# UmaimaKhan01/SkyEye-Aerial-Object-Detection-using-Yolo

Measured on AMD Instinct MI355X. Metric: frames/sec @1280x1280 + p50 latency, skyeye_s 1-GPU and skyeye_l 8-GPU, higher is better.
Workload: dtype bf16

## Files before the change

### skyeye-aerial-object-detection-using-yolo_amd/csrc/k_csp_stage.hip

```cpp
#include "sky_kernels.h"

#include "conv_frag.h"

namespace sky {

namespace cs {
constexpr int NW = 8, NT = NW * 64;
constexpr int TS = 16, HW = TS + 2, NHP = HW * HW;
constexpr int C = 64, HD = 32;
constexpr int XPIX = 352, XPL = XPIX * 32, X_BYTES = 4 * XPL;
constexpr int XDMA = XPIX / 32;
constexpr int HSL = 336, HPLN = HSL * 16, H_BYTES = 4 * HPLN;
constexpr int CPLN = 256 * 16, C_BYTES = 4 * CPLN;
constexpr int NFR = (NHP + 15) / 16;
constexpr int W12_BYTES = 2 * C * 64, WB1_BYTES = 1 * HD * 64, WB2_BYTES = 9 * HD * 64, W3_BYTES = 2 * C * 64;
constexpr int LDS_BYTES = X_BYTES + 2 * H_BYTES + C_BYTES + W12_BYTES + WB1_BYTES + WB2_BYTES + W3_BYTES + (C + HD + HD + C) * 4;
static_assert(LDS_BYTES <= 160 * 1024, "one workgroup per CU");
static_assert(HPLN % 256 == 0 && CPLN % 256 == 0 && XPL % 256 == 0, "planes a multiple of 256 B apart: conflict-free fragment reads");
}

__device__ __forceinline__ void cs_wait_vmcnt0() { __builtin_amdgcn_s_waitcnt(0x0F70); }
__device__ __forceinline__ void cs_lds_dma16(__amdgpu_buffer_rsrc_t rsrc, char* dst, int voff)
{
    __builtin_amdgcn_raw_ptr_buffer_load_lds(rsrc, (__attribute__((address_space(3))) void*)dst, 16, voff, 0, 0, 0);
}

template <int ROWS, int KSTEPS>
__device__ __forceinline__ void cs_stage_weights(const void* w, int kpad, char* lds, int tid)
{
    const char* src = reinterpret_cast<const char*>(w);
    for (int idx = tid; idx < KSTEPS * ROWS * 4; idx += cs::NT) {
        const int ks = idx / (ROWS * 4), rc = idx - ks * (ROWS * 4);
        const int rowp = rc >> 2, c = rc & 3;
        const int j = rowp >> 4, r = rowp & 15;
        const int ch = (j >> 1) * 32 + (r >> 2) * 8 + (j & 1) * 4 + (r & 3);
        const u32x4_t v = *reinterpret_cast<const u32x4_t*>(src + (long)ch * kpad * 2 + ks * 64 + c * 16);
        *reinterpret_cast<u32x4_t*>(lds + ks * (ROWS * 64) + rowp * 64 + ((c ^ (((r >> 3) & 1) << 1)) << 4)) = v;
    }
}

__global__ void __launch_bounds__(cs::NT) csp_stage_kernel(const CspStageArgs a)
{
    using namespace cs;
    extern __shared__ __attribute__((aligned(1024))) char smem[];
    char* const xt = smem;
    char* const y1t = xt + X_BYTES;
    char* const ut = y1t + H_BYTES;
    char* const y2t = ut + H_BYTES;
    char* const w12 = y2t + C_BYTES;
    char* const wb1 = w12 + W12_BYTES;
    char* const wb2 = wb1 + WB1_BYTES;
    char* const w3 = wb2 + WB2_BYTES;
    float* const b12 = reinterpret_cast<float*>(w3 + W3_BYTES);
    float* const bb1 = b12 + C;
    float* const bb2 = bb1 + HD;
    float* const b3 = bb2 + HD;

#ifdef SKY_AB_WAVE_VECTOR
    const int tid = threadIdx.x, lane = tid & 63, wave = tid >> 6;
#else
    const int tid = threadIdx.x, lane = tid & 63, wave = __builtin_amdgcn_readfirstlane(tid >> 6);
#endif
    const int fr = lane & 15, fq = lane >> 4;
    const int tiles_x = (a.W + TS - 1) / TS, tiles_y = (a.H + TS - 1) / TS;
    const int ntile = a.B * tiles_y * tiles_x;
    int tile, tstep, tend;
    tile_walk(ntile, tile, tstep, tend);
    if (tile >= tend) return;
    const int pix_b = a.ldi * 2;

    cs_stage_weights<C, 2>(a.w12, a.kpad12, w12, tid);
    cs_stage_weights<HD, 1>(a.wb1, a.kpadb1, wb1, tid);
    cs_stage_weights<HD, 9>(a.wb2, a.kpadb2, wb2, tid);
    cs_stage_weights<C, 2>(a.w3, a.kpad3, w3, tid);
    for (int i = tid; i < C; i += NT) { b12[i] = a.b12[i]; b3[i] = a.b3[i]; }
    for (int i = tid; i < HD; i += NT) { bb1[i] = a.bb1[i]; bb2[i] = a.bb2[i]; }

    const __amdgpu_buffer_rsrc_t irsrc = __builtin_amdgcn_make_buffer_rsrc(const_cast<void*>(a.in), 0, (int)a.in_bytes, 0x00020000);
    auto decode_tile = [&](int t, int& bimg, int& y0, int& x0) {
        const int tx = t % tiles_x;
        const int q = t / tiles_x;
        bimg = q / tiles_y;
        y0 = (q - bimg * tiles_y) * TS;
        x0 = tx * TS;
    };
    auto issue_x = [&](int bimg, int y0, int x0) {
        const int pl = wave & 3;
        const int base = ((bimg * a.H + y0 - 1) * a.W + x0 - 1) * pix_b + pl * 16;
        const int b0 = wave < 4 ? 0 : 6, b1 = wave < 4 ? 6 : XDMA;
        for (int b = b0; b < b1; ++b) {
            const int p = b * 32 + (lane >> 1);
            const int hy = (p * 3641) >> 16, hx = p - hy * HW;
            const int kk = (lane & 1) ^ ((p >> 3) & 1);
            const bool ok = p < NHP && (unsigned)(y0 - 1 + hy) < (unsigned)a.H && (unsigned)(x0 - 1 + hx) < (unsigned)a.W;
            cs_lds_dma16(irsrc, xt + pl * XPL + b * 1024, ok ? base + (hy * a.W + hx) * pix_b + kk * 64 : -1);
        }
    };
    const int aswz = ((fq ^ (((fr >> 3) & 1) << 1)) << 4);
    auto wfrag = [&](const char* w, int rows, int ks, int j) -> u32x4_t {
        return *reinterpret_cast<const u32x4_t*>(w + ks * (rows * 64) + (j * 16 + fr) * 64 + aswz);
    };
    auto xfrag = [&](int p, int kk) -> u32x4_t {
        return *reinterpret_cast<const u32x4_t*>(xt + fq * XPL + p * 32 + ((kk ^ ((p >> 3) & 1)) << 4));
    };
    auto act_pack = [&](const f32x4_t& a0, const f32x4_t& a1, float (&v)[8]) {
#pragma unroll
        for (int e = 0; e < 4; ++e) {
            v[e] = S1<__bf16>::silu(a0[e]);
            v[4 + e] = S1<__bf16>::silu(a1[e]);
        }
    };
    auto bias_pair = [&](const float* bias, f32x4_t& a0, f32x4_t& a1) {
        a0 = *reinterpret_cast<const f32x4_t*>(bias + fq * 8);
        a1 = *reinterpret_cast<const f32x4_t*>(bias + fq * 8 + 4);
    };

    int bimg, y0, x0;
    decode_tile(tile, bimg, y0, x0);
    __syncthreads();
#ifdef SKY_AB_SETPRIO
    if (__builtin_amdgcn_readfirstlane(tid >> 6) >= 4) __builtin_amdgcn_s_setprio(1);
#endif
    issue_x(bimg, y0, x0);
    for (;;) {
        cs_wait_vmcnt0();
        __syncthreads();
#pragma unroll 1
        for (int f = wave; f < NFR; f += NW) {
            const int p = f * 16 + fr;
            const int pc = p < NHP ? p : NHP - 1;
            const u32x4_t x0f = xfrag(pc, 0), x1f = xfrag(pc, 1);
            f32x4_t acc0, acc1;
            bias_pair(b12, acc0, acc1);
            S1<__bf16>::mma(wfrag(w12, C, 0, 0), x0f, acc0);
            S1<__bf16>::mma(wfrag(w12, C, 0, 1), x0f, acc1);
            S1<__bf16>::mma(wfrag(w12, C, 1, 0), x1f, acc0);
            S1<__bf16>::mma(wfrag(w12, C, 1, 1), x1f, acc1);
            float v[8];
            act_pack(acc0, acc1, v);
            const Out8<__bf16>::raw_t y1v = Out8<__bf16>::pack(v, 1.0f);
            f32x4_t au0, au1;
            bias_pair(bb1, au0, au1);
            S1<__bf16>::mma(wfrag(wb1, HD, 0, 0), y1v.a, au0);
            S1<__bf16>::mma(wfrag(wb1, HD, 0, 1), y1v.a, au1);
            act_pack(au0, au1, v);
            Out8<__bf16>::raw_t uv = Out8<__bf16>::pack(v, 1.0f);
            const int hy = (pc * 3641) >> 16, hx = pc - hy * HW;
            const bool inside = (unsigned)(y0 - 1 + hy) < (unsigned)a.H && (unsigned)(x0 - 1 + hx) < (unsigned)a.W;
            if (!inside) uv.a = u32x4_t{0u, 0u, 0u, 0u};
            if (p < NHP) {
                *reinterpret_cast<u32x4_t*>(y1t + fq * HPLN + p * 16) = y1v.a;
                *reinterpret_cast<u32x4_t*>(ut + fq * HPLN + p * 16) = uv.a;
            }
        }
#pragma unroll
        for (int i = 0; i < 2; ++i) {
            const int r = 2 * wave + i;
            const int p = (r + 1) * HW + 1 + fr;
            const u32x4_t x0f = xfrag(p, 0), x1f = xfrag(p, 1);
            f32x4_t acc0, acc1;
            bias_pair(b12 + HD, acc0, acc1);
            S1<__bf16>::mma(wfrag(w12, C, 0, 2), x0f, acc0);
            S1<__bf16>::mma(wfrag(w12, C, 0, 3), x0f, acc1);
            S1<__bf16>::mma(wfrag(w12, C, 1, 2), x1f, acc0);
            S1<__bf16>::mma(wfrag(w12, C, 1, 3), x1f, acc1);
            float v[8];
            act_pack(acc0, acc1, v);
            *reinterpret_cast<u32x4_t*>(y2t + fq * CPLN + (r * 16 + fr) * 16) = Out8<__bf16>::pack(v, 1.0f).a;
        }
        __syncthreads();
        const int next = tile + tstep;
        int nb = 0, ny0 = 0, nx0 = 0;
        if (next < tend) {
            decode_tile(next, nb, ny0, nx0);
            issue_x(nb, ny0, nx0);
        }
        {
            f32x4_t acc[2][2];
#pragma unroll
            for (int i = 0; i < 2; ++i) bias_pair(bb2, acc[0][i], acc[1][i]);
#pragma unroll
            for (int tap = 0; tap < 9; ++tap) {
                const int ky = tap / 3, kx = tap - ky * 3;
                u32x4_t pf[2];
#pragma unroll
                for (int i = 0; i < 2; ++i) pf[i] = *reinterpret_cast<const u32x4_t*>(ut + fq * HPLN + ((2 * wave + i + ky) * HW + fr + kx) * 16);
#pragma unroll
                for (int j = 0; j < 2; ++j) {
                    const u32x4_t wf = wfrag(wb2, HD, tap, j);
#pragma unroll
                    for (int i = 0; i < 2; ++i) S1<__bf16>::mma(wf, pf[i], acc[j][i]);
                }
            }
            f32x4_t acc3[4][2];
#pragma unroll
            for (int s = 0; s < 2; ++s)
#pragma unroll
                for (int i = 0; i < 2; ++i) bias_pair(b3 + s * 32, acc3[2 * s][i], acc3[2 * s + 1][i]);
            u32x4_t vv[2], y2v[2];
#pragma unroll
            for (int i = 0; i < 2; ++i) {
                const int r = 2 * wave + i;
                float v[8];
                if (a.shortcut) {
                    const Out8<__bf16>::raw_t rv = Out8<__bf16>::load(y1t + fq * HPLN + ((r + 1) * HW + 1 + fr) * 16);
#pragma unroll
                    for (int e = 0; e < 8; ++e) {
                        const float xx = e < 4 ? acc[0][i][e] : acc[1][i][e - 4];
                        const float t = S1<__bf16>::gate(xx);
                        const float res = (e & 1) ? __uint_as_float(rv.a[e >> 1] & 0xffff0000u) : __uint_as_float(rv.a[e >> 1] << 16);
                        v[e] = __builtin_fmaf(xx, t, res);
                    }
                } else {
                    act_pack(acc[0][i], acc[1][i], v);
                }
                vv[i] = Out8<__bf16>::pack(v, 1.0f).a;
                y2v[i] = *reinterpret_cast<const u32x4_t*>(y2t + fq * CPLN + (r * 16 + fr) * 16);
            }
#pragma unroll
            for (int j = 0; j < 4; ++j) {
                const u32x4_t wf = wfrag(w3, C, 0, j);
#pragma unroll
                for (int i = 0; i < 2; ++i) S1<__bf16>::mma(wf, vv[i], acc3[j][i]);
            }
#pragma unroll
            for (int j = 0; j < 4; ++j) {
                const u32x4_t wf = wfrag(w3, C, 1, j);
#pragma unroll
                for (int i = 0; i < 2; ++i) S1<__bf16>::mma(wf, y2v[i], acc3[j][i]);
            }
#pragma unroll
            for (int i = 0; i < 2; ++i) {
                const int oy = y0 + 2 * wave + i, ox = x0 + fr;
                if (oy < a.H && ox < a.W) {
                    char* op = reinterpret_cast<char*>(a.out) + (((long)bimg * a.H + oy) * a.W + ox) * (long)a.ldo * 2;
#pragma unroll
                    for (int s = 0; s < 2; ++s) {
                        float v[8];
                        act_pack(acc3[2 * s][i], acc3[2 * s + 1][i], v);
                        Out8<__bf16>::store(Out8<__bf16>::pack(v, 1.0f), op + (s * 32 + fq * 8) * 2);
                    }
                }
            }
        }
        if (next >= tend) break;
        tile = next; bimg = nb; y0 = ny0; x0 = nx0;
    }
}

bool csp_stage_supported(const CspStageArgs& a)
{
    return a.c == cs::C && a.hidden == cs::HD && a.ldi % 8 == 0 && a.ldo % 8 == 0 && a.in_bytes != 0 && a.kpad12 >= cs::C && a.kpadb1 >= cs::HD &&
           a.kpadb2 >= 9 * cs::HD && a.kpad3 >= cs::C && a.H >= 1 && a.W >= 1 && !(a.opts & OPT_NO_CSP_STAGE);
}

hipError_t launch_csp_stage(const CspStageArgs& a, hipStream_t s)
{
    if (!csp_stage_supported(a)) return hipErrorNotSupported;
    static size_t attr[16] = {0};
    {
        const hipError_t e = ensure_lds_attr(reinterpret_cast<const void*>(csp_stage_kernel), cs::LDS_BYTES, a.device, attr);
        if (e != hipSuccess) return e;
    }
    const int ntile = a.B * ((a.H + cs::TS - 1) / cs::TS) * ((a.W + cs::TS - 1) / cs::TS);
    const int n_cu = a.n_cu > 0 ? a.n_cu : 256;
    const int gx = ntile < n_cu ? ntile : n_cu;
    hipLaunchKernelGGL(csp_stage_kernel, dim3(gx), dim3(cs::NT), cs::LDS_BYTES, s, a);
    return hipGetLastError();
}

}
```

### skyeye-aerial-object-detection-using-yolo_amd/csrc/k_stem_down.hip

```cpp
#include "sky_kernels.h"

#include "conv_frag.h"

namespace sky {

namespace sd {
constexpr int NW = 8;
constexpr int NT = NW * 64;
constexpr int C1 = 32, C2 = 64;
constexpr int TS = 16;
constexpr int SS = 2 * TS + 1;
constexpr int HS = SS + 2;
constexpr int RS = 2 * HS;
constexpr int RDW = (2 * HS + 2) / 4;
constexpr int RAWP = RDW * 4;
constexpr int RAW_BYTES = 3 * RS * RAWP;
constexpr int NDW = (3 * RS * RDW + NT - 1) / NT;
constexpr int S2D_SLOTS = (HS * HS + 15) / 16 * 16;
constexpr int S2D_PLANE = S2D_SLOTS * 16;
constexpr int S2D_BYTES = 2 * S2D_PLANE;
constexpr int NPIX = (S2D_SLOTS + NT - 1) / NT;
constexpr int PC00 = 304, PC01 = 272, PC10 = 272, PC11 = 256;
constexpr int PB00 = 0, PB01 = PB00 + 4 * PC00 * 16 + 64, PB10 = PB01 + 4 * PC01 * 16 + 64, PB11 = PB10 + 4 * PC10 * 16 + 64;
constexpr int STEM_BYTES = PB11 + 4 * PC11 * 16 + 64;
static_assert(PB00 % 128 == 0 && PB10 % 128 == 0 && PB01 % 128 == 64 && PB11 % 128 == 64, "odd-column planes 64 bytes off the even ones");
static_assert(STEM_BYTES % 256 == 0, "the space-to-depth tile behind the stem tile stays 256-byte aligned");
constexpr int KS1 = 5;
constexpr int W1_BYTES = KS1 * C1 * 64;
constexpr int W2_BYTES = 9 * C2 * 64;
constexpr int NPF = (SS * SS + 15) / 16;
constexpr int PFW = (NPF + NW - 1) / NW;
constexpr int LDS_BYTES = STEM_BYTES + S2D_BYTES + W1_BYTES + W2_BYTES + (C1 + C2) * 4;
static_assert(RAW_BYTES <= STEM_BYTES, "the raw blocks are staged inside the (not yet written) stem tile");
static_assert(LDS_BYTES <= 160 * 1024, "one workgroup per CU");
static_assert(PFW % 3 == 0, "phase B walks the fragments of a wave in groups of three");

__device__ __forceinline__ int pcells(int par) { return par == 0 ? PC00 : par == 1 ? PC01 : par == 2 ? PC10 : PC11; }
__device__ __forceinline__ int pbase(int par) { return par == 0 ? PB00 : par == 1 ? PB01 : par == 2 ? PB10 : PB11; }
__device__ __forceinline__ int ppitch(int par) { return (par & 1) ? 16 : 17; }
}

template <int ROWS, int KSTEPS>
__device__ __forceinline__ void sd_stage_weights(const void* w, int kpad, int kbytes, char* lds, int tid)
{
    const char* src = reinterpret_cast<const char*>(w);
    for (int idx = tid; idx < KSTEPS * ROWS * 4; idx += sd::NT) {
        const int ks = idx / (ROWS * 4), rc = idx - ks * (ROWS * 4);
        const int rowp = rc >> 2, c = rc & 3;
        const int j = rowp >> 4, r = rowp & 15;
        const int ch = (j >> 1) * 32 + (r >> 2) * 8 + (j & 1) * 4 + (r & 3);
        const int kb = ks * 64 + c * 16;
        u32x4_t v = {0u, 0u, 0u, 0u};
        if (kb < kbytes) v = *reinterpret_cast<const u32x4_t*>(src + (long)ch * kpad * 2 + kb);
        *reinterpret_cast<u32x4_t*>(lds + ks * (ROWS * 64) + rowp * 64 + ((c ^ (((r >> 3) & 1) << 1)) << 4)) = v;
    }
}

__device__ __forceinline__ bool stem_pixel(int f, int fr, int& sy, int& sx)
{
    using namespace sd;
    if (f < 2 * SS) {
        sy = f >> 1;
        sx = (f & 1) * 16 + fr;
        return true;
    }
    sy = (f - 2 * SS) * 16 + fr;
    sx = SS - 1;
    const bool real = f < NPF && sy < SS;
    if (!real) sy = SS - 1;
    return real;
}

__global__ void __launch_bounds__(sd::NT) stem_down_kernel(const StemDownArgs a)
{
    using namespace sd;
    extern __shared__ __attribute__((aligned(1024))) char smem[];
    char* const stem = smem;
    unsigned char* const rawl = reinterpret_cast<unsigned char*>(smem);
    char* const s2d = smem + STEM_BYTES;
    char* const w1 = s2d + S2D_BYTES;
    char* const w2 = w1 + W1_BYTES;
    float* const b1 = reinterpret_cast<float*>(w2 + W2_BYTES);
    float* const b2 = b1 + C1;

    const int tid = threadIdx.x, lane = tid & 63, wave = tid >> 6;
    const int fr = lane & 15, fq = lane >> 4;
    const int Hs = a.Hr / 2, Ws = a.Wr / 2;
    const int tiles_x = (a.Wo + TS - 1) / TS, tiles_y = (a.Ho + TS - 1) / TS;
    const int ntile = a.B * tiles_y * tiles_x;
    int tile, tstep, tend;
    tile_walk(ntile, tile, tstep, tend);
    if (tile >= tend) return;

    sd_stage_weights<C1, KS1>(a.w1, a.kpad1, 9 * 32, w1, tid);
    sd_stage_weights<C2, 9>(a.w2, a.kpad2, 9 * 64, w2, tid);
    for (int i = tid; i < C1; i += NT) b1[i] = a.bias1[i];
    for (int i = tid; i < C2; i += NT) b2[i] = a.bias2[i];

    auto decode_tile = [&](int t, int& bimg, int& y0, int& x0) {
        const int tx = t % tiles_x;
        const int q = t / tiles_x;
        bimg = q / tiles_y;
        y0 = (q - bimg * tiles_y) * TS;
        x0 = tx * TS;
    };
    unsigned int rawd[NDW];
    auto load_raw = [&](int t) {
        int bimg, y0, x0;
        decode_tile(t, bimg, y0, x0);
        const int ry0 = 4 * y0 - 4, rx0 = 4 * x0 - 4;
#pragma unroll
        for (int k = 0; k < NDW; ++k) {
            const int d = tid + k * NT;
            unsigned int v = 0u;
            if (d < 3 * RS * RDW) {
                const int r = d / RDW, cd = d - r * RDW;
                const int col = r / RS, ry = r - col * RS;
                const int y = ry0 + ry, x = rx0 + 4 * cd;
                if ((unsigned)y < (unsigned)a.Hr && x >= 0 && x + 3 < a.Wr)
                    v = *reinterpret_cast<const unsigned int*>(a.frames + (((long)bimg * 3 + col) * a.Hr + y) * a.Wr + x);
            }
            rawd[k] = v;
        }
    };
    int toff[KS1];
#pragma unroll
    for (int ks = 0; ks < KS1; ++ks) {
        const int c = ks * 4 + fq;
        int tap = c >> 1;
        if (tap > 8) tap = 8;
        const int ky = (tap * 11) >> 5, kx = tap - ky * 3;
        toff[ks] = (c & 1) * S2D_PLANE + (ky * HS + kx) * 16;
    }
    const int aswz = ((fq ^ (((fr >> 3) & 1) << 1)) << 4);

    load_raw(tile);
    __syncthreads();
#ifdef SKY_AB_SETPRIO
    if (__builtin_amdgcn_readfirstlane(threadIdx.x >> 6) >= 4) __builtin_amdgcn_s_setprio(1);
#endif
    for (;;) {
        int bimg, y0, x0;
        decode_tile(tile, bimg, y0, x0);
#pragma unroll
        for (int k = 0; k < NDW; ++k) {
            const int d = tid + k * NT;
            if (d < 3 * RS * RDW) *reinterpret_cast<unsigned int*>(rawl + d * 4) = rawd[k];
        }
        __syncthreads();
#pragma unroll 1
        for (int k = 0; k < NPIX; ++k) {
            const int p = tid + k * NT;
            if (p < S2D_SLOTS) {
                const int hy = p / HS, hx = p - hy * HS;
                const int gy = 2 * y0 - 2 + hy, gx = 2 * x0 - 2 + hx;
                const bool inside = p < HS * HS && (unsigned)gy < (unsigned)Hs && (unsigned)gx < (unsigned)Ws;
                const int hyc = p < HS * HS ? hy : 0;
                float f[16];
#pragma unroll
                for (int col = 0; col < 3; ++col)
#pragma unroll
                    for (int dy = 0; dy < 2; ++dy) {
                        const unsigned int two = *reinterpret_cast<const unsigned short*>(rawl + (col * RS + 2 * hyc + dy) * RAWP + 2 * hx);
                        f[dy * 3 + col] = (float)(two & 255u) * (1.0f / 255.0f);
                        f[6 + dy * 3 + col] = (float)(two >> 8) * (1.0f / 255.0f);
                    }
#pragma unroll
                for (int e = 12; e < 16; ++e) f[e] = 0.0f;
                u32x4_t o0, o1;
#pragma unroll
                for (int e = 0; e < 4; ++e) {
                    o0[e] = inside ? pack_bf16x2(f[2 * e], f[2 * e + 1]) : 0u;
                    o1[e] = inside ? pack_bf16x2(f[8 + 2 * e], f[8 + 2 * e + 1]) : 0u;
                }
                *reinterpret_cast<u32x4_t*>(s2d + p * 16) = o0;
                *reinterpret_cast<u32x4_t*>(s2d + S2D_PLANE + p * 16) = o1;
            }
        }
        __syncthreads();
        const int next = tile + tstep;
        if (next < tend) load_raw(next);

        const f32x4_t bia0 = *reinterpret_cast<const f32x4_t*>(b1 + fq * 8);
        const f32x4_t bia1 = *reinterpret_cast<const f32x4_t*>(b1 + fq * 8 + 4);
        auto gemm3 = [&](int g3, f32x4_t (&acc)[2][3]) {
            int pb[3];
#pragma unroll
            for (int i = 0; i < 3; ++i) {
                int sy, sx;
                stem_pixel(wave * PFW + g3 * 3 + i, fr, sy, sx);
                pb[i] = (sy * HS + sx) * 16;
                acc[0][i] = bia0;
                acc[1][i] = bia1;
            }
#pragma unroll
            for (int ks = 0; ks < KS1; ++ks) {
                const u32x4_t wf0 = *reinterpret_cast<const u32x4_t*>(w1 + ks * (C1 * 64) + fr * 64 + aswz);
                const u32x4_t wf1 = *reinterpret_cast<const u32x4_t*>(w1 + ks * (C1 * 64) + (16 + fr) * 64 + aswz);
#pragma unroll
                for (int i = 0; i < 3; ++i) {
                    const u32x4_t pf = *reinterpret_cast<const u32x4_t*>(s2d + pb[i] + toff[ks]);
                    S1<__bf16>::mma(wf0, pf, acc[0][i]);
                    S1<__bf16>::mma(wf1, pf, acc[1][i]);
                }
            }
        };
        auto act3 = [&](int g3, const f32x4_t (&acc)[2][3]) {
#pragma unroll
            for (int i = 0; i < 3; ++i) {
                int sy, sx;
                const bool real = stem_pixel(wave * PFW + g3 * 3 + i, fr, sy, sx);
                const int gy = 2 * y0 - 1 + sy, gx = 2 * x0 - 1 + sx;
                const bool inside = (unsigned)gy < (unsigned)Hs && (unsigned)gx < (unsigned)Ws;
                float v[8];
#pragma unroll
                for (int e = 0; e < 4; ++e) {
                    v[e] = S1<__bf16>::silu(acc[0][i][e]);
                    v[4 + e] = S1<__bf16>::silu(acc[1][i][e]);
                }
                Out8<__bf16>::raw_t o = Out8<__bf16>::pack(v, 1.0f);
                if (!inside) o.a = u32x4_t{0u, 0u, 0u, 0u};
                const int par = (sy & 1) * 2 + (sx & 1);
                const int cell = (sy >> 1) * ppitch(par) + (sx >> 1);
                if (real) *reinterpret_cast<u32x4_t*>(stem + pbase(par) + fq * (pcells(par) * 16) + cell * 16) = o.a;
            }
        };
        {
            f32x4_t accA[2][3], accB[2][3];
            gemm3(0, accA);
            gemm3(1, accB);
            act3(0, accA);
            gemm3(2, accA);
            act3(1, accB);
            act3(2, accA);
        }
        __syncthreads();

        {
            f32x4_t acc[4][2];
#pragma unroll
            for (int j = 0; j < 4; ++j) {
                const f32x4_t c = *reinterpret_cast<const f32x4_t*>(b2 + (j >> 1) * 32 + fq * 8 + (j & 1) * 4);
#pragma unroll
                for (int i = 0; i < 2; ++i) acc[j][i] = c;
            }
#pragma unroll
            for (int tap = 0; tap < 9; ++tap) {
                const int ky = tap / 3, kx = tap - ky * 3;
                const int par = (ky & 1) * 2 + (kx & 1);
                const char* pl = stem + pbase(par) + fq * (pcells(par) * 16);
                u32x4_t pf[2];
#pragma unroll
                for (int i = 0; i < 2; ++i) {
                    const int y = 2 * wave + i;
                    pf[i] = *reinterpret_cast<const u32x4_t*>(pl + ((y + (ky >> 1)) * ppitch(par) + fr + (kx >> 1)) * 16);
                }
#pragma unroll
                for (int j = 0; j < 4; ++j) {
                    const u32x4_t wf = *reinterpret_cast<const u32x4_t*>(w2 + tap * (C2 * 64) + (j * 16 + fr) * 64 + aswz);
#pragma unroll
                    for (int i = 0; i < 2; ++i) S1<__bf16>::mma(wf, pf[i], acc[j][i]);
                }
            }
#pragma unroll
            for (int i = 0; i < 2; ++i) {
                const int oy = y0 + 2 * wave + i, ox = x0 + fr;
                if (oy < a.Ho && ox < a.Wo) {
                    char* op = reinterpret_cast<char*>(a.out) + (((long)bimg * a.Ho + oy) * a.Wo + ox) * (long)a.ldo * 2;
#pragma unroll
                    for (int s = 0; s < 2; ++s) {
                        float v[8];
#pragma unroll
                        for (int e = 0; e < 4; ++e) {
                            v[e] = S1<__bf16>::silu(acc[2 * s][i][e]);
                            v[4 + e] = S1<__bf16>::silu(acc[2 * s + 1][i][e]);
                        }
                        Out8<__bf16>::store(Out8<__bf16>::pack(v, 1.0f), op + (s * 32 + fq * 8) * 2);
                    }
                }
            }
        }
        if (next >= tend) break;
        tile = next;
        __syncthreads();
    }
}

bool stem_down_supported(const StemDownArgs& a)
{
    return a.c1 == sd::C1 && a.c2 == sd::C2 && a.Hr % 2 == 0 && a.Wr % 4 == 0 && a.kpad1 * 2 >= 9 * 32 && a.kpad2 * 2 >= 9 * 64 &&
           a.ldo % 8 == 0 && (double)a.B * 3.0 * a.Hr * a.Wr < 2147483000.0 && !(a.opts & OPT_NO_STEM_DOWN);
}

hipError_t launch_stem_down(const StemDownArgs& a, hipStream_t s)
{
    if (!stem_down_supported(a)) return hipErrorNotSupported;
    static size_t attr[16] = {0};
    {
        const hipError_t e = ensure_lds_attr(reinterpret_cast<const void*>(stem_down_kernel), sd::LDS_BYTES, a.device, attr);
        if (e != hipSuccess) return e;
    }
    const int ntile = a.B * ((a.Ho + sd::TS - 1) / sd::TS) * ((a.Wo + sd::TS - 1) / sd::TS);
    const int n_cu = a.n_cu > 0 ? a.n_cu : 256;
    const int gx = ntile < n_cu ? ntile : n_cu;
    hipLaunchKernelGGL(stem_down_kernel, dim3(gx), dim3(sd::NT), sd::LDS_BYTES, s, a);
    return hipGetLastError();
}

}
```

Measured before the change: 7671.

## Add interior-tile fast paths and split stem conv2 into two pipelined halves

Adds an interior-tile test to the CSP-stage and stem-down kernels. Interior tiles use precomputed per-thread buffer offsets for the DMA and raw loads and skip the per-pixel boundary masking. The stem kernel also gets a specialised stem-store path for regular fragments and a scalarised wave index. Its second 3x3 conv is restructured into two output-channel halves: all tap fragments are loaded up front, the SiLU of the first half is interleaved with the MMAs of the second, weight fragments are prefetched, and sched barriers enforce the order. This raises register pressure and adds code paths that must stay consistent with the edge logic.

```diff
diff --git a/skyeye-aerial-object-detection-using-yolo_amd/csrc/k_csp_stage.hip b/skyeye-aerial-object-detection-using-yolo_amd/csrc/k_csp_stage.hip
--- a/skyeye-aerial-object-detection-using-yolo_amd/csrc/k_csp_stage.hip
+++ b/skyeye-aerial-object-detection-using-yolo_amd/csrc/k_csp_stage.hip
@@ -84,10 +84,32 @@
         y0 = (q - bimg * tiles_y) * TS;
         x0 = tx * TS;
     };
+    auto interior = [&](int y0, int x0) {
+#ifdef SKY_ISA_INTERIOR
+        return true;
+#endif
+        return y0 >= 1 && x0 >= 1 && y0 + TS + 1 <= a.H && x0 + TS + 1 <= a.W;
+    };
+    const int xb0 = wave < 4 ? 0 : 6, xnb = wave < 4 ? 6 : XDMA - 6;
+    int xoff[6];
+#pragma unroll
+    for (int i = 0; i < 6; ++i) {
+        const int p = (xb0 + i) * 32 + (lane >> 1);
+        const int hy = (p * 3641) >> 16, hx = p - hy * HW;
+        const int kk = (lane & 1) ^ ((p >> 3) & 1);
+        xoff[i] = p < NHP ? (hy * a.W + hx) * pix_b + kk * 64 + (wave & 3) * 16 : -1;
+    }
     auto issue_x = [&](int bimg, int y0, int x0) {
         const int pl = wave & 3;
+        const int b0 = wave < 4 ? 0 : 6, b1 = wave < 4 ? 6 : XDMA;
+        if (interior(y0, x0)) {
+            const int tb = ((bimg * a.H + y0 - 1) * a.W + x0 - 1) * pix_b;
+#pragma unroll
+            for (int i = 0; i < 6; ++i)
+                if (i < xnb) cs_lds_dma16(irsrc, xt + pl * XPL + (xb0 + i) * 1024, xoff[i] < 0 ? -1 : tb + xoff[i]);
+            return;
+        }
         const int base = ((bimg * a.H + y0 - 1) * a.W + x0 - 1) * pix_b + pl * 16;
-        const int b0 = wave < 4 ? 0 : 6, b1 = wave < 4 ? 6 : XDMA;
         for (int b = b0; b < b1; ++b) {
             const int p = b * 32 + (lane >> 1);
             const int hy = (p * 3641) >> 16, hx = p - hy * HW;
@@ -125,11 +147,11 @@
     for (;;) {
         cs_wait_vmcnt0();
         __syncthreads();
+        const bool tin = interior(y0, x0);
 #pragma unroll 1
         for (int f = wave; f < NFR; f += NW) {
             const int p = f * 16 + fr;
-            const int pc = p < NHP ? p : NHP - 1;
-            const u32x4_t x0f = xfrag(pc, 0), x1f = xfrag(pc, 1);
+            const u32x4_t x0f = xfrag(p, 0), x1f = xfrag(p, 1);
             f32x4_t acc0, acc1;
             bias_pair(b12, acc0, acc1);
             S1<__bf16>::mma(wfrag(w12, C, 0, 0), x0f, acc0);
@@ -145,9 +167,11 @@
             S1<__bf16>::mma(wfrag(wb1, HD, 0, 1), y1v.a, au1);
             act_pack(au0, au1, v);
             Out8<__bf16>::raw_t uv = Out8<__bf16>::pack(v, 1.0f);
-            const int hy = (pc * 3641) >> 16, hx = pc - hy * HW;
-            const bool inside = (unsigned)(y0 - 1 + hy) < (unsigned)a.H && (unsigned)(x0 - 1 + hx) < (unsigned)a.W;
-            if (!inside) uv.a = u32x4_t{0u, 0u, 0u, 0u};
+            if (!tin) {
+                const int hy = (p * 3641) >> 16, hx = p - hy * HW;
+                const bool inside = (unsigned)(y0 - 1 + hy) < (unsigned)a.H && (unsigned)(x0 - 1 + hx) < (unsigned)a.W;
+                if (!inside) uv.a = u32x4_t{0u, 0u, 0u, 0u};
+            }
             if (p < NHP) {
                 *reinterpret_cast<u32x4_t*>(y1t + fq * HPLN + p * 16) = y1v.a;
                 *reinterpret_cast<u32x4_t*>(ut + fq * HPLN + p * 16) = uv.a;
diff --git a/skyeye-aerial-object-detection-using-yolo_amd/csrc/k_stem_down.hip b/skyeye-aerial-object-detection-using-yolo_amd/csrc/k_stem_down.hip
--- a/skyeye-aerial-object-detection-using-yolo_amd/csrc/k_stem_down.hip
+++ b/skyeye-aerial-object-detection-using-yolo_amd/csrc/k_stem_down.hip
@@ -83,7 +83,7 @@
     float* const b1 = reinterpret_cast<float*>(w2 + W2_BYTES);
     float* const b2 = b1 + C1;
 
-    const int tid = threadIdx.x, lane = tid & 63, wave = tid >> 6;
+    const int tid = threadIdx.x, lane = tid & 63, wave = __builtin_amdgcn_readfirstlane(tid >> 6);
     const int fr = lane & 15, fq = lane >> 4;
     const int Hs = a.Hr / 2, Ws = a.Wr / 2;
     const int tiles_x = (a.Wo + TS - 1) / TS, tiles_y = (a.Ho + TS - 1) / TS;
@@ -104,11 +104,33 @@
         y0 = (q - bimg * tiles_y) * TS;
         x0 = tx * TS;
     };
+    auto interior = [&](int y0, int x0) {
+#ifdef SKY_ISA_INTERIOR
+        return true;
+#endif
+        return y0 >= 1 && x0 >= 1 && 4 * y0 + RS - 4 <= a.Hr && 4 * x0 + RAWP - 4 <= a.Wr && y0 + TS <= a.Ho && x0 + TS <= a.Wo;
+    };
+    int roff[NDW];
+#pragma unroll
+    for (int k = 0; k < NDW; ++k) {
+        const int d = tid + k * NT;
+        const int r = d / RDW, cd = d - r * RDW;
+        const int col = r / RS, ry = r - col * RS;
+        roff[k] = d < 3 * RS * RDW ? (col * a.Hr + ry) * a.Wr + 4 * cd : 0;
+    }
+    const __amdgpu_buffer_rsrc_t frsrc = __builtin_amdgcn_make_buffer_rsrc(const_cast<unsigned char*>(a.frames), 0,
+                                                                           (int)((long)a.B * 3 * a.Hr * a.Wr), 0x00020000);
     unsigned int rawd[NDW];
     auto load_raw = [&](int t) {
         int bimg, y0, x0;
         decode_tile(t, bimg, y0, x0);
         const int ry0 = 4 * y0 - 4, rx0 = 4 * x0 - 4;
+        if (interior(y0, x0)) {
+            const int sbase = (bimg * 3 * a.Hr + ry0) * a.Wr + rx0;
+#pragma unroll
+            for (int k = 0; k < NDW; ++k) rawd[k] = __builtin_amdgcn_raw_buffer_load_b32(frsrc, roff[k], sbase, 0);
+            return;
+        }
 #pragma unroll
         for (int k = 0; k < NDW; ++k) {
             const int d = tid + k * NT;
@@ -133,6 +155,9 @@
         toff[ks] = (c & 1) * S2D_PLANE + (ky * HS + kx) * 16;
     }
     const int aswz = ((fq ^ (((fr >> 3) & 1) << 1)) << 4);
+    const int prow0 = (fr & 1) ? PB01 + fq * (PC01 * 16) + (fr >> 1) * 16 : PB00 + fq * (PC00 * 16) + (fr >> 1) * 16;
+    const int prow1 = (fr & 1) ? PB11 + fq * (PC11 * 16) + (fr >> 1) * 16 : PB10 + fq * (PC10 * 16) + (fr >> 1) * 16;
+    const int podd = (fr & 1) ? 0 : 16;
 
     load_raw(tile);
     __syncthreads();
@@ -142,6 +167,7 @@
     for (;;) {
         int bimg, y0, x0;
         decode_tile(tile, bimg, y0, x0);
+        const bool tin = interior(y0, x0);
 #pragma unroll
         for (int k = 0; k < NDW; ++k) {
             const int d = tid + k * NT;
@@ -154,7 +180,7 @@
             if (p < S2D_SLOTS) {
                 const int hy = p / HS, hx = p - hy * HS;
                 const int gy = 2 * y0 - 2 + hy, gx = 2 * x0 - 2 + hx;
-                const bool inside = p < HS * HS && (unsigned)gy < (unsigned)Hs && (unsigned)gx < (unsigned)Ws;
+                const bool inside = p < HS * HS && (tin || ((unsigned)gy < (unsigned)Hs && (unsigned)gx < (unsigned)Ws));
                 const int hyc = p < HS * HS ? hy : 0;
                 float f[16];
 #pragma unroll
@@ -208,10 +234,7 @@
         auto act3 = [&](int g3, const f32x4_t (&acc)[2][3]) {
 #pragma unroll
             for (int i = 0; i < 3; ++i) {
-                int sy, sx;
-                const bool real = stem_pixel(wave * PFW + g3 * 3 + i, fr, sy, sx);
-                const int gy = 2 * y0 - 1 + sy, gx = 2 * x0 - 1 + sx;
-                const bool inside = (unsigned)gy < (unsigned)Hs && (unsigned)gx < (unsigned)Ws;
+                const int f = wave * PFW + g3 * 3 + i;
                 float v[8];
 #pragma unroll
                 for (int e = 0; e < 4; ++e) {
@@ -219,10 +242,24 @@
                     v[4 + e] = S1<__bf16>::silu(acc[1][i][e]);
                 }
                 Out8<__bf16>::raw_t o = Out8<__bf16>::pack(v, 1.0f);
-                if (!inside) o.a = u32x4_t{0u, 0u, 0u, 0u};
-                const int par = (sy & 1) * 2 + (sx & 1);
-                const int cell = (sy >> 1) * ppitch(par) + (sx >> 1);
-                if (real) *reinterpret_cast<u32x4_t*>(stem + pbase(par) + fq * (pcells(par) * 16) + cell * 16) = o.a;
+                if (f < 2 * SS) {
+                    const int sy = f >> 1;
+                    if (!tin) {
+                        const int gy = 2 * y0 - 1 + sy, gx = 2 * x0 - 1 + (f & 1) * 16 + fr;
+                        if (!((unsigned)gy < (unsigned)Hs && (unsigned)gx < (unsigned)Ws)) o.a = u32x4_t{0u, 0u, 0u, 0u};
+                    }
+                    const int off = ((sy & 1) ? prow1 : prow0) + (sy >> 1) * (16 * 16) + (f & 1) * (8 * 16) + (sy >> 1) * podd;
+                    *reinterpret_cast<u32x4_t*>(stem + off) = o.a;
+                } else {
+                    int sy, sx;
+                    const bool real = stem_pixel(f, fr, sy, sx);
+                    const int gy = 2 * y0 - 1 + sy, gx = 2 * x0 - 1 + sx;
+                    const bool inside = (unsigned)gy < (unsigned)Hs && (unsigned)gx < (unsigned)Ws;
+                    if (!inside) o.a = u32x4_t{0u, 0u, 0u, 0u};
+                    const int par = (sy & 1) * 2 + (sx & 1);
+                    const int cell = (sy >> 1) * ppitch(par) + (sx >> 1);
+                    if (real) *reinterpret_cast<u32x4_t*>(stem + pbase(par) + fq * (pcells(par) * 16) + cell * 16) = o.a;
+                }
             }
         };
         {
@@ -237,46 +274,76 @@
         __syncthreads();
 
         {
-            f32x4_t acc[4][2];
-#pragma unroll
-            for (int j = 0; j < 4; ++j) {
-                const f32x4_t c = *reinterpret_cast<const f32x4_t*>(b2 + (j >> 1) * 32 + fq * 8 + (j & 1) * 4);
-#pragma unroll
-                for (int i = 0; i < 2; ++i) acc[j][i] = c;
-            }
+            u32x4_t pf[9][2];
 #pragma unroll
             for (int tap = 0; tap < 9; ++tap) {
                 const int ky = tap / 3, kx = tap - ky * 3;
                 const int par = (ky & 1) * 2 + (kx & 1);
                 const char* pl = stem + pbase(par) + fq * (pcells(par) * 16);
-                u32x4_t pf[2];
 #pragma unroll
                 for (int i = 0; i < 2; ++i) {
                     const int y = 2 * wave + i;
-                    pf[i] = *reinterpret_cast<const u32x4_t*>(pl + ((y + (ky >> 1)) * ppitch(par) + fr + (kx >> 1)) * 16);
-                }
-#pragma unroll
-                for (int j = 0; j < 4; ++j) {
-                    const u32x4_t wf = *reinterpret_cast<const u32x4_t*>(w2 + tap * (C2 * 64) + (j * 16 + fr) * 64 + aswz);
-#pragma unroll
-                    for (int i = 0; i < 2; ++i) S1<__bf16>::mma(wf, pf[i], acc[j][i]);
-                }
+                    pf[tap][i] = *reinterpret_cast<const u32x4_t*>(pl + ((y + (ky >> 1)) * ppitch(par) + fr + (kx >> 1)) * 16);
+                }
+            }
+            auto wfrag2 = [&](int tap, int j) { return *reinterpret_cast<const u32x4_t*>(w2 + tap * (C2 * 64) + (j * 16 + fr) * 64 + aswz); };
+            auto bias2 = [&](int s, f32x4_t (&acc)[2][2]) {
+#pragma unroll
+                for (int jj = 0; jj < 2; ++jj) {
+                    const f32x4_t c = *reinterpret_cast<const f32x4_t*>(b2 + s * 32 + fq * 8 + jj * 4);
+#pragma unroll
+                    for (int i = 0; i < 2; ++i) acc[jj][i] = c;
+                }
+            };
+            f32x4_t acc0[2][2], acc1[2][2];
+            bias2(0, acc0);
+#pragma unroll
+            for (int tap = 0; tap < 9; ++tap)
+#pragma unroll
+                for (int jj = 0; jj < 2; ++jj) {
+                    const u32x4_t wf = wfrag2(tap, jj);
+#pragma unroll
+                    for (int i = 0; i < 2; ++i) S1<__bf16>::mma(wf, pf[tap][i], acc0[jj][i]);
+                }
+            bias2(1, acc1);
+            float h0[16];
+            u32x4_t wn[2] = {wfrag2(0, 2), wfrag2(0, 3)};
+#pragma unroll
+            for (int tap = 0; tap < 9; ++tap) {
+                const u32x4_t wc[2] = {wn[0], wn[1]};
+                if (tap < 8) { wn[0] = wfrag2(tap + 1, 2); wn[1] = wfrag2(tap + 1, 3); }
+#pragma unroll
+                for (int jj = 0; jj < 2; ++jj)
+#pragma unroll
+                    for (int i = 0; i < 2; ++i) S1<__bf16>::mma(wc[jj], pf[tap][i], acc1[jj][i]);
+                if (tap < 8) {
+#pragma unroll
+                    for (int q = 2 * tap; q < 2 * tap + 2; ++q) {
+                        h0[q] = S1<__bf16>::silu(acc0[(q >> 2) & 1][q >> 3][q & 3]);
+                        asm volatile("" ::"v"(h0[q]));
+                    }
+                }
+                __builtin_amdgcn_sched_barrier(0);
+            }
+            u32x4_t o[2][2];
+#pragma unroll
+            for (int i = 0; i < 2; ++i) {
+                o[0][i] = Out8<__bf16>::pack(&h0[8 * i], 1.0f).a;
+                float v[8];
+#pragma unroll
+                for (int e = 0; e < 4; ++e) {
+                    v[e] = S1<__bf16>::silu(acc1[0][i][e]);
+                    v[4 + e] = S1<__bf16>::silu(acc1[1][i][e]);
+                }
+                o[1][i] = Out8<__bf16>::pack(v, 1.0f).a;
             }
 #pragma unroll
             for (int i = 0; i < 2; ++i) {
                 const int oy = y0 + 2 * wave + i, ox = x0 + fr;
-                if (oy < a.Ho && ox < a.Wo) {
+                if (tin || (oy < a.Ho && ox < a.Wo)) {
                     char* op = reinterpret_cast<char*>(a.out) + (((long)bimg * a.Ho + oy) * a.Wo + ox) * (long)a.ldo * 2;
 #pragma unroll
-                    for (int s = 0; s < 2; ++s) {
-                        float v[8];
-#pragma unroll
-                        for (int e = 0; e < 4; ++e) {
-                            v[e] = S1<__bf16>::silu(acc[2 * s][i][e]);
-                            v[4 + e] = S1<__bf16>::silu(acc[2 * s + 1][i][e]);
-                        }
-                        Out8<__bf16>::store(Out8<__bf16>::pack(v, 1.0f), op + (s * 32 + fq * 8) * 2);
-                    }
+                    for (int s = 0; s < 2; ++s) *reinterpret_cast<u32x4_t*>(op + (s * 32 + fq * 8) * 2) = o[s][i];
                 }
             }
         }
```

New measurement: 7778 (median of 6 runs). 1.01x the previous value.
